# Socrates666/esp32-wake-word

Measured on AMD Instinct MI355X. Metric: audio windows/sec (1s@16kHz, 40-MFCC) through xiaoa CNN at 1/2/4/8 MI355X, higher is better.
Workload: dtype f32; 1 GPU; config2: fused MFCC(torchaudio+CMVN)+xiaoa CNN fp32, B clips per GPU; audio=fp32 samples, batch_per_gpu=65536, global_batch=65536, seq_len=16000, parallelism=dp1 (per-rank clip split, no collectives), process_group_world_size=1

## Files before the change

### esp32-wake-word_amd/csrc/wk_fused.hip

```cpp
#include "wk_fused_dev.h"

namespace {

#ifdef WK_DIAG
__device__ unsigned long long g_wk_stamps[16][16];
#endif

constexpr int kCnnCarve = kImgEnd - kGOff;
constexpr int kCnnLds = 2 * kCnnCarve;
static_assert(kCnnLds * 4 <= 163840, "standalone CNN LDS budget");
static_assert(kCnnCarve % 4 == 0 && kGOff % 4 == 0, "16-byte aligned carves");

template <int CM>
__global__ __launch_bounds__(kFusedBlock, 4) void wk_cnn_fused_kernel(const float* __restrict__ feats, int64_t batch,
                                                                     const float* __restrict__ wts,
                                                                     const uint16_t* __restrict__ wbf,
                                                                     float* __restrict__ logits, unsigned* err) {
  __shared__ __attribute__((aligned(16))) float smem[kCnnLds];
  const int tid = threadIdx.x, lane = tid & 63;
  const int wave = __builtin_amdgcn_readfirstlane(tid >> 6);
  for (int i = tid; i < kCnnLds; i += kFusedBlock) smem[i] = 0.0f;
  __syncthreads();
  const int role = wave >> 3;
  float* base = smem + role * kCnnCarve - kGOff;
  const int64_t cb = 2 * (int64_t)blockIdx.x + role, cs = 2 * (int64_t)gridDim.x;
  const int64_t n_mine = batch > cb ? (batch - 1 - cb) / cs + 1 : 0;
  FeatSrc<CM> src = {feats, base, cb, cs, 0};
  cnn_role<CM>(base, wts, wbf, n_mine, cb, cs, logits, wave & 7, lane, src);
  report_abort(reinterpret_cast<const unsigned*>(base + kCtrlOff), err, lane);
}

}

#ifdef WK_DIAG
extern "C" int wk_debug_stamps(unsigned long long* host_out, int reset) {
  if (hipMemcpyFromSymbol(host_out, HIP_SYMBOL(g_wk_stamps), sizeof(g_wk_stamps)) != hipSuccess) return 1;
  if (reset) {
    static unsigned long long zero[16][16];
    if (hipMemcpyToSymbol(HIP_SYMBOL(g_wk_stamps), zero, sizeof(zero)) != hipSuccess) return 1;
  }
  return 0;
}
#endif

namespace wk {

hipError_t launch_fused(bool i16, const void* audio, int64_t batch, int64_t clip_stride, const float* w,
                        const uint16_t* wbf, int conv_mode, float* logits, float* feats_or_null, int grid_cap,
                        hipStream_t stream, unsigned* err, int diag) {
  if (batch == 0) return hipSuccess;
  if (conv_mode != kConvF32 && !wbf) return hipErrorInvalidValue;
#ifdef WK_DIAG
  return launch_fused_modes<kConvBf16, kConvBf16x3, kConvF32>(i16, conv_mode, audio, batch, clip_stride, w, wbf, logits,
                                                              feats_or_null, grid_cap, stream, err, diag);
#else
  if (conv_mode != kConvF32)
    return launch_fused_xdl(i16, audio, batch, clip_stride, w, wbf, conv_mode, logits, feats_or_null, grid_cap, stream,
                            err, diag);
  return launch_fused_modes<kConvF32>(i16, conv_mode, audio, batch, clip_stride, w, wbf, logits, feats_or_null,
                                      grid_cap, stream, err, diag);
#endif
}

hipError_t launch_cnn_fused(const float* feats, int64_t batch, const float* w, const uint16_t* wbf, int conv_mode,
                            float* logits, int grid_cap, hipStream_t stream, unsigned* err) {
  if (batch == 0) return hipSuccess;
  if (conv_mode != kConvF32 && !wbf) return hipErrorInvalidValue;
  const int64_t roles = (batch + NBF - 1) / NBF;
  const int grid = (int)((roles + 1) / 2 < grid_cap ? (roles + 1) / 2 : grid_cap);
  if (conv_mode == kConvBf16)
    hipLaunchKernelGGL(wk_cnn_fused_kernel<kConvBf16>, dim3(grid), dim3(kFusedBlock), 0, stream, feats, batch, w, wbf,
                       logits, err);
  else if (conv_mode == kConvBf16x3)
    hipLaunchKernelGGL(wk_cnn_fused_kernel<kConvBf16x3>, dim3(grid), dim3(kFusedBlock), 0, stream, feats, batch, w,
                       wbf, logits, err);
  else
    hipLaunchKernelGGL(wk_cnn_fused_kernel<kConvF32>, dim3(grid), dim3(kFusedBlock), 0, stream, feats, batch, w, wbf,
                       logits, err);
  return hipGetLastError();
}

}
```

### esp32-wake-word_amd/csrc/wk_fused_cnn_role.h

```cpp
#pragma once
#include "wk_fused_lds.h"
#include "wk_cnn_dev.h"
#include "wk_kernels.h"

namespace {

__device__ __forceinline__ float row_sum16(float v) {
  v += dpp<0xB1>(v);
  v += dpp<0x4E>(v);
  v += dpp<0x141>(v);
  v += dpp<0x140>(v);
  return v;
}

template <int CM>
__device__ __forceinline__ void dct_cmvn_clip(const float* __restrict__ lbuf, int slot, float* __restrict__ F0,
                                              uint16_t* __restrict__ B0, uint16_t* __restrict__ X0,
                                              float* __restrict__ fo, int lane) {
  const int li = lane & 15, lk = lane >> 4;
  int aoff = 48 * lane;
  asm volatile("" : "+v"(aoff));
  const auto ra = make_rsrc(kDctB16, sizeof(kDctB16));
  float dA[12];
#pragma unroll
  for (int s = 0; s < 12; s += 4) {
    const f32x4 v = __builtin_bit_cast(f32x4, __builtin_amdgcn_raw_buffer_load_b128(ra, aoff, 4 * s, 0));
#pragma unroll
    for (int r = 0; r < 4; ++r) dA[s + r] = v[r];
  }
  f32x4 d[4] = {{0, 0, 0, 0}, {0, 0, 0, 0}, {0, 0, 0, 0}, {0, 0, 0, 0}};
#pragma unroll
  for (int s = 0; s < 10; ++s) {
    const f32x4 b = *reinterpret_cast<const f32x4*>(lbuf + (4 * s + lk) * WK_LSTRIDE + 4 * li);
#pragma unroll
    for (int nt = 0; nt < 4; ++nt) d[nt] = mfma4(dA[s], b[nt], d[nt]);
  }
  const bool v3 = li != 15;
  const int row0 = lane & 48;
#pragma unroll
  for (int r = 0; r < 4; ++r) {
    const float a = d[0][r];
    const float nx = __int_as_float(__builtin_amdgcn_update_dpp(__float_as_int(a), __float_as_int(a), 0x101, 0xF, 0xF, false));
    const bool ne = (a != d[1][r]) | (a != d[2][r]) | (v3 & (a != d[3][r])) | (a != nx);
    const bool flat = ((__builtin_amdgcn_ballot_w64(ne) >> row0) & 0xFFFFull) == 0;
#pragma unroll
    for (int nt = 0; nt < 4; ++nt) d[nt][r] = flat ? 0.0f : d[nt][r];
  }
  float mean[4], inv[4];
#pragma unroll
  for (int r = 0; r < 4; ++r) {
    const float x3 = v3 ? d[3][r] : 0.0f;
    mean[r] = row_sum16((d[0][r] + d[1][r]) + (d[2][r] + x3)) * (1.0f / kNFramesB);
    float dv[4];
#pragma unroll
    for (int nt = 0; nt < 4; ++nt) dv[nt] = d[nt][r] - mean[r];
    dv[3] = v3 ? dv[3] : 0.0f;
    const float q = row_sum16((dv[0] * dv[0] + dv[1] * dv[1]) + (dv[2] * dv[2] + dv[3] * dv[3]));
    float sd = __builtin_amdgcn_sqrtf(q * (1.0f / (kNFramesB - 1)));
    sd = sd == 0.0f ? 1.0f : sd;
    inv[r] = __builtin_amdgcn_rcpf(sd + 1e-8f);
  }
#pragma unroll
  for (int nt = 0; nt < 4; ++nt) {
    const int t = 4 * li + nt;
    if (nt == 3 && !v3) continue;
    const int row = slot * I0_TP + 1 + t;
    float y[4];
#pragma unroll
    for (int r = 0; r < 4; ++r) y[r] = (d[nt][r] - mean[r]) * inv[r];
    if constexpr (CM == kConvBf16) {
      uint2 pk;
      pk.x = bf16_bits(y[0]) | (bf16_bits(y[1]) << 16);
      pk.y = bf16_bits(y[2]) | (bf16_bits(y[3]) << 16);
      *reinterpret_cast<uint2*>(B0 + row * I0_CIP + 4 * lk) = pk;
    } else if constexpr (CM == kConvBf16x3) {
      uint32_t h[4], l[4];
#pragma unroll
      for (int r = 0; r < 4; ++r) {
        h[r] = bf16_bits(y[r]);
        l[r] = bf16_bits(y[r] - __uint_as_float(h[r] << 16));
      }
      *reinterpret_cast<uint2*>(X0 + row * X0_CIP + 4 * lk) = make_uint2(h[0] | (h[1] << 16), h[2] | (h[3] << 16));
      *reinterpret_cast<uint2*>(X0 + row * X0_CIP + 16 + 4 * lk) = make_uint2(l[0] | (l[1] << 16), l[2] | (l[3] << 16));
    } else {
      *reinterpret_cast<f32x4*>(F0 + row * F0_CIP + 4 * lk) = f32x4{y[0], y[1], y[2], y[3]};
    }
    if (fo) {
#pragma unroll
      for (int r = 0; r < 4; ++r)
        if (4 * lk + r < 13) fo[(4 * lk + r) * kNFramesB + t] = y[r];
    }
  }
}

template <int CM, class SRC>
__device__ __forceinline__ void cnn_role(float* base, const float* __restrict__ pk, const uint16_t* __restrict__ pkb,
                                         int64_t n_mine, int64_t clip_base, int64_t clip_step,
                                         float* __restrict__ logits, int cw, int lane, SRC& src) {
  float* F0 = base + kF0Off;
  float* F1 = base + kF1Off;
  float* F2 = base + kF2Off;
  uint16_t* B0 = reinterpret_cast<uint16_t*>(base + kB0Off);
  uint16_t* B1 = reinterpret_cast<uint16_t*>(base + kB1Off);
  uint16_t* B2 = reinterpret_cast<uint16_t*>(base + kB2Off);
  uint16_t* X0 = reinterpret_cast<uint16_t*>(base + kX0Off);
  uint16_t* X1 = reinterpret_cast<uint16_t*>(base + kX1Off);
  uint16_t* X2 = reinterpret_cast<uint16_t*>(base + kX2Off);
  constexpr bool BF = CM == kConvBf16, X3 = CM == kConvBf16x3;
  constexpr int kLoW = kNumPackedBf16;
  const auto rsb = make_rsrc(pkb, 2 * kNumPackedBf16 * (X3 ? 2 : 1));
  auto frag_bf = [&](int elem_off) -> s8 {
    return __builtin_bit_cast(s8, __builtin_amdgcn_raw_buffer_load_b128(rsb, 16 * lane, 2 * elem_off, 0));
  };
  float* Gp = base + kGOff;
  float* FCP = base + kFcpOff;
  unsigned* ctrl = reinterpret_cast<unsigned*>(base + kCtrlOff);
  const int li = lane & 15, lk = lane >> 4;
  unsigned gen = 0;
  const auto rs = make_rsrc(pk, 4 * kNumPacked);

  auto load_frags = [&](auto& w, int first) {
    constexpr int n = sizeof(w) / sizeof(float);
    static_assert(n % 4 == 0, "whole groups of four k-steps");
#pragma unroll
    for (int s = 0; s < n; s += 4) {
      const f32x4 v = __builtin_bit_cast(f32x4, __builtin_amdgcn_raw_buffer_load_b128(rs, 16 * lane, 4 * (first + s * 64), 0));
#pragma unroll
      for (int r = 0; r < 4; ++r) w[s + r] = v[r];
    }
  };
  float w3[48];
  s8 w3b[6];
  if constexpr (BF || X3) {
#pragma unroll
    for (int s = 0; s < 6; ++s) w3b[s] = frag_bf(kPbW3 + (cw * 6 + s) * kBfFrag);
  }
  if constexpr (CM == kConvF32) load_frags(w3, kPkW3 + cw * 48 * 64);
  const int64_t n_batches = (n_mine + NBF - 1) / NBF;
  src.init(cw, lane);
  bool eager_done = false;
  auto try_eager = [&](int64_t b) {
    if (cw >= NBF || eager_done) return;
    const int64_t i = (b + 1) * NBF + cw;
    if (i >= n_mine) return;
    if (src.ready(i)) {
      src.load(i, cw);
      eager_done = true;
    }
  };
  auto fc2 = [&](int64_t bb) {
    if (cw != 0) return;
    int ln = lane;
    asm volatile("" : "+v"(ln));
    const int cl = ln & (NBF - 1), q = ln >> 2;
    float h[4];
    if constexpr (CM == kConvF32) {
      f32x4 v = *reinterpret_cast<const f32x4*>(FCP + cl * 64 + 4 * q);
#pragma unroll
      for (int w = 1; w < 8; ++w) v += *reinterpret_cast<const f32x4*>(FCP + (w * NBF + cl) * 64 + 4 * q);
#pragma unroll
      for (int r = 0; r < 4; ++r) h[r] = v[r];
    } else {
      const f32x4 v = *reinterpret_cast<const f32x4*>(FCP + cl * 64 + 4 * q);
#pragma unroll
      for (int r = 0; r < 4; ++r) h[r] = v[r];
#pragma unroll
      for (int w = 1; w < 8; ++w) {
        const f32x4 u = *reinterpret_cast<const f32x4*>(FCP + (w * NBF + cl) * 64 + 4 * q);
#pragma unroll
        for (int r = 0; r < 4; ++r) h[r] += u[r];
      }
    }
    float acc = 0.0f;
#pragma unroll
    for (int i2 = 0; i2 < 4; ++i2) acc = __builtin_fmaf(buf_load(rs, 16 * q, 4 * (kPkF2 + i2)), fmaxf(h[i2], 0.0f), acc);
    acc += __shfl_xor(acc, 4, 64);
    acc += __shfl_xor(acc, 8, 64);
    acc += __shfl_xor(acc, 16, 64);
    acc += __shfl_xor(acc, 32, 64);
    const int64_t i = bb * NBF + cl;
    if (q == 0 && i < n_mine) logits[clip_base + clip_step * i] = acc;
  };
  WK_STAMP_INIT
  for (int64_t b = 0; b < n_batches; ++b) {
    if (cw < NBF && !eager_done) {
      const int64_t i = b * NBF + cw;
      if (i < n_mine) {
        src.wait(i);
        src.load(i, cw);
      }
    }
    eager_done = false;
    float w1[12];
    s8 w1b[2], w1l[2];
    if constexpr (BF || X3) {
#pragma unroll
      for (int s = 0; s < 2; ++s) w1b[s] = frag_bf(kPbW1 + ((cw & 1) * 2 + s) * kBfFrag);
    }
    if constexpr (X3) {
#pragma unroll
      for (int s = 0; s < 2; ++s) w1l[s] = frag_bf(kLoW + kPbW1 + ((cw & 1) * 2 + s) * kBfFrag);
    }
    if constexpr (CM == kConvF32) load_frags(w1, kPkW1 + (cw & 1) * 12 * 64);
    WK_STAMP(0);
    role_sync<0>(ctrl, kCtrlCnnBar, gen, lane);
    if (b > 0) fc2(b - 1);

    const int nv = n_mine - b * NBF < NBF ? (int)(n_mine - b * NBF) : NBF;

    if ((cw >> 1) < nv) {
      const int co0 = 16 * (cw & 1), cl = cw >> 1;
      const int bo = (cl * I0_TP + li) * I0_CIP;
#pragma unroll 1
      for (int p = 0; p < 2; ++p) {
        const int ta = 32 * p, tb = ta + 16;
        f32x4 acc_a = {0, 0, 0, 0}, acc_b = {0, 0, 0, 0};
        if constexpr (BF) {
          conv_pair_bf<2, 16, I0_CIP>(B0, w1b, bo + ta * I0_CIP, bo + tb * I0_CIP, lk, acc_a, acc_b);
          epi_pool_bf<I1_CIP, I1_TP, 31>(acc_a, B1, co0, cl, ta, lane);
          epi_pool_bf<I1_CIP, I1_TP, 31>(acc_b, B1, co0, cl, tb, lane);
        } else if constexpr (X3) {
          const int bx = (cl * I0_TP + li) * X0_CIP;
          conv_pair_bf3<2, 16, X0_CIP>(X0, w1b, w1l, bx + ta * X0_CIP, bx + tb * X0_CIP, lk, acc_a, acc_b);
          epi_pool_bf3<X1_CIP, I1_TP, 31, 32>(acc_a, X1, co0, cl, ta, lane);
          epi_pool_bf3<X1_CIP, I1_TP, 31, 32>(acc_b, X1, co0, cl, tb, lane);
        } else {
          f32x4 m[4] = {{0, 0, 0, 0}, {0, 0, 0, 0}, {0, 0, 0, 0}, {0, 0, 0, 0}};
          conv_wino_v<1, F0_CIP>(F0, w1, (cl * I0_TP + 2 * (16 * p + li)) * F0_CIP + 4 * lk, m);
          epi_wino_pool<F1_CIP, I1_TP, 31>(m, F1, co0, cl, 16 * p, lane);
        }
      }
    }
    WK_STAMP(1);
    role_sync<0>(ctrl, kCtrlCnnBar, gen, lane);
    try_eager(b);
    WK_STAMP(2);

    if constexpr (BF) {
      s8 w2b[3];
#pragma unroll
      for (int s = 0; s < 3; ++s) w2b[s] = frag_bf(kPbW2 + ((cw & 3) * 3 + s) * kBfFrag);
      const int co0 = 16 * (cw & 3);
#pragma unroll 1
      for (int p = 0; p < 2; ++p) {
        const int cl = 2 * (cw >> 2) + p;
        if (cl >= nv) break;
        const int bb = (cl * I1_TP + li) * I1_CIP;
        f32x4 acc_a = {0, 0, 0, 0}, acc_b = {0, 0, 0, 0};
        conv_pair_bf<3, 32, I1_CIP>(B1, w2b, bb, bb + 16 * I1_CIP, lk, acc_a, acc_b);
        epi_pool_bf<I2_CIP, I2_TP, 15>(acc_a, B2, co0, cl, 0, lane);
        epi_pool_bf<I2_CIP, I2_TP, 15>(acc_b, B2, co0, cl, 16, lane);
      }
    } else if constexpr (X3) {
      s8 w2b[3], w2l[3];
#pragma unroll
      for (int s = 0; s < 3; ++s) w2b[s] = frag_bf(kPbW2 + ((cw & 3) * 3 + s) * kBfFrag);
#pragma unroll
      for (int s = 0; s < 3; ++s) w2l[s] = frag_bf(kLoW + kPbW2 + ((cw & 3) * 3 + s) * kBfFrag);
      const int co0 = 16 * (cw & 3);
#pragma unroll 1
      for (int p = 0; p < 2; ++p) {
        const int cl = 2 * (cw >> 2) + p;
        if (cl >= nv) break;
        const int bb = (cl * I1_TP + li) * X1_CIP;
        f32x4 acc_a = {0, 0, 0, 0}, acc_b = {0, 0, 0, 0};
        conv_pair_bf3<3, 32, X1_CIP>(X1, w2b, w2l, bb, bb + 16 * X1_CIP, lk, acc_a, acc_b);
        epi_pool_bf3<X2_CIP, I2_TP, 15, 64>(acc_a, X2, co0, cl, 0, lane);
        epi_pool_bf3<X2_CIP, I2_TP, 15, 64>(acc_b, X2, co0, cl, 16, lane);
      }
    } else {
      float w2[24];
      load_frags(w2, kPkW2 + (cw & 3) * 24 * 64);
      const int co0 = 16 * (cw & 3);
#pragma unroll 1
      for (int p = 0; p < 2; ++p) {
        const int cl = 2 * (cw >> 2) + p;
        if (cl >= nv) break;
        f32x4 m[4] = {{0, 0, 0, 0}, {0, 0, 0, 0}, {0, 0, 0, 0}, {0, 0, 0, 0}};
        conv_wino_v<2, F1_CIP, 1>(F1, w2, (cl * I1_TP + 2 * li) * F1_CIP + 4 * lk, m);
        epi_wino_pool<F2_CIP, I2_TP, 15>(m, F2, co0, cl, 0, lane);
      }
    }
    WK_STAMP(3);
    role_sync<0>(ctrl, kCtrlCnnBar, gen, lane);
    try_eager(b);
    WK_STAMP(4);

    {
      const int co0 = 16 * cw;
      const int bo = li * I2_CIP;
#pragma unroll 1
      for (int p = 0; p < 2; ++p) {
        if (p > 0) try_eager(b);
        const int ca = 2 * p, cb = 2 * p + 1;
        if (ca >= nv) break;
        f32x4 acc_a = {0, 0, 0, 0}, acc_b = {0, 0, 0, 0};
        if constexpr (BF) {
          conv_pair_bf<6, 64, I2_CIP, 3>(B2, w3b, bo + ca * I2_TP * I2_CIP, bo + cb * I2_TP * I2_CIP, lk, acc_a,
                                         acc_b);
        } else if constexpr (X3) {
          s8 w3l[6];
#pragma unroll
          for (int s = 0; s < 6; ++s) w3l[s] = frag_bf(kLoW + kPbW3 + (cw * 6 + s) * kBfFrag);
          const int bx = li * X2_CIP;
          conv_pair_bf3<6, 64, X2_CIP, 2>(X2, w3b, w3l, bx + ca * I2_TP * X2_CIP, bx + cb * I2_TP * X2_CIP, lk,
                                          acc_a, acc_b);
        } else {
          f32x4 m[4] = {{0, 0, 0, 0}, {0, 0, 0, 0}, {0, 0, 0, 0}, {0, 0, 0, 0}};
          conv_wino_v<4, F2_CIP, 1>(F2, w3, ((ca + (li >> 3)) * I2_TP + 2 * (li & 7)) * F2_CIP + 4 * lk, m);
          epi_wino_gap<NBF>(m, Gp, co0, ca, lane);
          continue;
        }
        epi_gap<NBF>(acc_a, Gp, co0, ca, lane);
        epi_gap<NBF>(acc_b, Gp, co0, cb, lane);
      }
    }
    float wf1[16];
    load_frags(wf1, kPkF1 + cw * 16 * 64);
    WK_STAMP(5);
    role_sync<0>(ctrl, kCtrlCnnBar, gen, lane);
    try_eager(b);
    WK_STAMP(6);

    {
      int ln = lane;
      asm volatile("" : "+v"(ln));
      f32x4 acc = {0, 0, 0, 0};
      const float* g = Gp + 16 * cw * NBF + (ln & (NBF - 1));
#pragma unroll
      for (int s = 0; s < 16; ++s) acc = mfma4x4(wf1[s], g[s * NBF], acc);
      *reinterpret_cast<f32x4*>(FCP + (cw * NBF + (ln & (NBF - 1))) * 64 + 4 * (ln >> 2)) = acc;
    }
    try_eager(b);
    WK_STAMP(8);
  }
  if (n_batches > 0) {
    role_sync<0>(ctrl, kCtrlCnnBar, gen, lane);
    fc2(n_batches - 1);
  }
  WK_STAMP_FLUSH(8 + cw);
}

template <int CM, bool FEATS>
struct LogmelSrc {
  float* smem;
  unsigned* ctrl;
  float* feats_out;
  int64_t clip_base, clip_step;
  int cw, lane, diag;
  __device__ __forceinline__ void init(int cw_, int lane_) {
    cw = cw_;
    lane = lane_;
    signal_set(ctrl, kCtrlLFree + cw, cw < NBF ? (unsigned)cw : 0xFFFFFFFFu, lane);
  }
  __device__ __forceinline__ bool ready(int64_t i) const {
    __atomic_signal_fence(__ATOMIC_SEQ_CST);
    const bool r = (diag & 2) ||
                   __builtin_amdgcn_readfirstlane(lds_load(ctrl + kCtrlLReady)) >= 8u * (unsigned)(i + 1);
    asm volatile("" ::: "memory");
    __atomic_signal_fence(__ATOMIC_SEQ_CST);
    return r;
  }
  __device__ __forceinline__ void wait(int64_t i) const {
    if (!(diag & 2)) spin_until<0>(ctrl, kCtrlLReady, 8u * (unsigned)(i + 1));
  }
  __device__ __forceinline__ void load(int64_t i, int slot) const {
    float* fo = FEATS ? feats_out + (clip_base + clip_step * i) * (13 * kNFramesB) : nullptr;
    dct_cmvn_clip<CM>(smem + (i & 1 ? kL1Off : kLOff), slot, smem + kF0Off,
                      reinterpret_cast<uint16_t*>(smem + kB0Off), reinterpret_cast<uint16_t*>(smem + kX0Off), fo,
                      lane);
    signal_set(ctrl, kCtrlLFree + cw, (unsigned)(i + NBF), lane);
  }
};

template <int CM>
struct FeatSrc {
  const float* feats;
  float* base;
  int64_t clip_base, clip_step;
  int lane;
  __device__ __forceinline__ void init(int, int lane_) { lane = lane_; }
  __device__ __forceinline__ bool ready(int64_t) const { return true; }
  __device__ __forceinline__ void wait(int64_t) const {}
  __device__ __forceinline__ void load(int64_t i, int slot) const {
    const float* f = feats + (clip_base + clip_step * i) * (13 * kNFramesB);
    if (lane >= kNFramesB) return;
    float y[13];
#pragma unroll
    for (int c = 0; c < 13; ++c) y[c] = __builtin_nontemporal_load(f + c * kNFramesB + lane);
    const int row = slot * I0_TP + 1 + lane;
    if constexpr (CM == kConvBf16) {
      uint16_t* B0 = reinterpret_cast<uint16_t*>(base + kB0Off) + row * I0_CIP;
#pragma unroll
      for (int c = 0; c < 12; c += 4)
        *reinterpret_cast<uint2*>(B0 + c) = make_uint2(bf16_bits(y[c]) | (bf16_bits(y[c + 1]) << 16),
                                                       bf16_bits(y[c + 2]) | (bf16_bits(y[c + 3]) << 16));
      B0[12] = (uint16_t)bf16_bits(y[12]);
    } else if constexpr (CM == kConvBf16x3) {
      uint16_t* X0 = reinterpret_cast<uint16_t*>(base + kX0Off) + row * X0_CIP;
#pragma unroll
      for (int c = 0; c < 13; ++c) {
        const uint32_t h = bf16_bits(y[c]);
        X0[c] = (uint16_t)h;
        X0[16 + c] = (uint16_t)bf16_bits(y[c] - __uint_as_float(h << 16));
      }
    } else {
      float* F0 = base + kF0Off + row * F0_CIP;
#pragma unroll
      for (int c = 0; c < 12; c += 4) *reinterpret_cast<f32x4*>(F0 + c) = f32x4{y[c], y[c + 1], y[c + 2], y[c + 3]};
      F0[12] = y[12];
    }
  }
};

}
```

### esp32-wake-word_amd/csrc/wk_fused_dev.h

```cpp
#pragma once
#include "wk_fused_lds.h"
#include "wk_fused_fe_role.h"
#include "wk_fused_cnn_role.h"
#include "wk_kernels.h"
#include <type_traits>

namespace {

template <typename T, int CM, bool FEATS>
__global__ __launch_bounds__(kFusedBlock, 4) void wk_fused_kernel(const T* __restrict__ audio, int64_t batch,
                                                                 int64_t clip_stride, const float* __restrict__ wts,
                                                                 const uint16_t* __restrict__ wbf,
                                                                 float* __restrict__ logits,
                                                                 float* __restrict__ feats_out, unsigned* err,
                                                                 int diag) {
  __shared__ __attribute__((aligned(16))) float smem[kFusedLds];
#ifndef WK_DIAG
  diag = 0;
#endif
  const int tid = threadIdx.x;
  const int lane = tid & 63;
  const int wave = __builtin_amdgcn_readfirstlane(tid >> 6);
  typedef std::conditional_t<CM == kConvF32, FePacked, FeScalar> FE;
  fe_init_tables<true, true, FE>(smem, tid, kFusedBlock);
  for (int i = tid; i < kFusedLds - kGOff; i += kFusedBlock) smem[kGOff + i] = 0.0f;
  __syncthreads();
  const int64_t n_mine = batch > (int64_t)blockIdx.x ? (batch - 1 - blockIdx.x) / gridDim.x + 1 : 0;
  if (wave < kFeWaves) __builtin_amdgcn_s_setprio(kPrioFe);
  if (wave < kFeWaves) {
    if (!(diag & 2)) fe_role<T, FE>(smem, audio, n_mine, clip_stride, wave, lane, diag);
  } else {
    if (!(diag & 1)) {
      LogmelSrc<CM, FEATS> src = {smem, reinterpret_cast<unsigned*>(smem + kCtrlOff), feats_out, (int64_t)blockIdx.x,
                                  (int64_t)gridDim.x, 0, 0, diag};
      cnn_role<CM>(smem, wts, wbf, n_mine, (int64_t)blockIdx.x, (int64_t)gridDim.x, logits, wave - kFeWaves, lane,
                   src);
    }
  }
  report_abort(reinterpret_cast<unsigned*>(smem + kCtrlOff), err, lane);
}

template <typename T, int CM>
hipError_t launch_fused_as(const void* audio, int64_t batch, int64_t clip_stride, const float* w, const uint16_t* wbf,
                           float* logits, float* feats_or_null, int grid_cap, hipStream_t stream, unsigned* err,
                           int diag) {
  const dim3 g((int)(batch < grid_cap ? batch : grid_cap)), blk(kFusedBlock);
  if (feats_or_null)
    hipLaunchKernelGGL((wk_fused_kernel<T, CM, true>), g, blk, 0, stream, (const T*)audio, batch, clip_stride, w, wbf,
                       logits, feats_or_null, err, diag);
  else
    hipLaunchKernelGGL((wk_fused_kernel<T, CM, false>), g, blk, 0, stream, (const T*)audio, batch, clip_stride, w, wbf,
                       logits, nullptr, err, diag);
  return hipGetLastError();
}

template <typename T, int CM, int... REST, typename... A>
hipError_t launch_fused_mode(int conv_mode, A... a) {
  if constexpr (sizeof...(REST) > 0)
    return conv_mode == CM ? launch_fused_as<T, CM>(a...) : launch_fused_mode<T, REST...>(conv_mode, a...);
  else
    return launch_fused_as<T, CM>(a...);
}
template <int... CMS, typename... A>
hipError_t launch_fused_modes(bool i16, int conv_mode, A... a) {
  return i16 ? launch_fused_mode<int16_t, CMS...>(conv_mode, a...) : launch_fused_mode<float, CMS...>(conv_mode, a...);
}

}
```

### esp32-wake-word_amd/csrc/wk_fused_fe_role.h

```cpp
#pragma once
#include "wk_fused_lds.h"

namespace {

template <typename T, typename FE>
__device__ __forceinline__ void fe_role(float* smem, const T* __restrict__ audio, int64_t n_mine,
                                        int64_t clip_stride, int wave, int lane, int diag) {
  float* P = smem + kPOff;
  float* L = smem + kLOff;
  float* L1 = smem + kL1Off;
  unsigned* ctrl = reinterpret_cast<unsigned*>(smem + kCtrlOff);
  const int g = lane >> 4, j = lane & 15;
  const FeTables tb = fe_tables(smem, j, nullptr);
  const int slot_base = fe_lds::slot_base(g);
  const int64_t G = gridDim.x;
  unsigned gen = 0, p_wait = 0;

  const int64_t step = G * clip_stride;
  const T* cptr = audio + (int64_t)blockIdx.x * clip_stride;
  constexpr uint32_t kClipBytes = kWinSamples * sizeof(T);
  struct PfCtx {
    __amdgpu_buffer_rsrc_t rs;
    int base;
    int xb;
  };
  auto fwr = [&](int r) { return FE::round1_swap && r == 1 ? wave ^ 4 : wave; };
  auto pf_ctx = [&](const T* p, bool ok, int r) -> PfCtx {
    const int fl = fwr(r) + fe_lds::kRoundSlots * r + slot_base;
    return {make_rsrc(p, ok ? kClipBytes : 0u), 256 * fl - 160, fl == 0 ? 160 : 256 * fl - 161};
  };

  Raw<T> pf;
  {
    const PfCtx c0 = pf_ctx(cptr, n_mine > 0, 0);
#pragma unroll
    for (int k = 0; k < 4; ++k) load_raw_part<FE>(c0.rs, c0.base, c0.xb, j, pf, k);
  }
  WK_STAMP_INIT
  for (int64_t i = 0; i < n_mine; ++i) {
#pragma unroll 1
    for (int r = 0; r <= 1; ++r) {
      const int fl = fwr(r) + fe_lds::kRoundSlots * r + slot_base;
      const int edge = r == 0 && fwr(r) == 0 ? 1 : r == 1 && fwr(r) == 6 ? 2 : 0;
      typename FE::c2 a[16];
#ifdef WK_DIAG
      asm volatile("s_waitcnt vmcnt(0)" ::: "memory");
      WK_STAMP(11);
#endif
      fe_stage0_fused(pf, lane, edge, tb, a);
      WK_STAMP(0);
      const PfCtx nx = r < 1 ? pf_ctx(cptr, true, r + 1) : pf_ctx(cptr + step, i + 1 < n_mine, 0);
      auto pf_part = [&](int k) {
        if (k >= 0) {
          load_raw_part<FE>(nx.rs, nx.base, nx.xb, j, pf, k);
        } else if (r == 0) {
          spin_until<kPrioFe>(ctrl, kCtrlFeBar, p_wait);
          WK_STAMP(9);
        }
      };
      WK_STAMP(1);
      float* row = fl < kNFramesB ? P + fl * kPRow : smem + kDummyRowOff;
      fe_rest<true, FE>(a, j, row, tb, 0, pf_part WK_SP_ARG);
    }
    role_sync<kPrioFe>(ctrl, kCtrlFeBar, gen, lane);
    WK_STAMP(7);
    if (i >= 2 && !(diag & 1)) spin_until_all8<kPrioFe>(ctrl, kCtrlLFree, (unsigned)(i - 1));
    WK_STAMP(10);
    {
      int prow = kPOff + min(lane, kNFramesB - 1) * kPRow;
      asm volatile("" : "+v"(prow));
      mel_dispatch<true>(wave, smem + prow, (i & 1 ? L1 : L) + lane);
      WK_STAMP(8);
      signal_add(ctrl, kCtrlLReady, lane);
    }
    gen += 8;
    signal_add(ctrl, kCtrlFeBar, lane);
    p_wait = gen;
    cptr += step;
  }
  WK_STAMP_FLUSH(wave);
}

}
```

### esp32-wake-word_amd/csrc/wk_fused_lds.h

```cpp
#pragma once
#include "wk_fe_dev.h"

using namespace wk;

namespace {

#ifdef WK_DIAG
extern __device__ unsigned long long g_wk_stamps[16][16];
#define WK_STAMP_INIT WkStamps _stamps; _stamps.init();
#define WK_STAMP(k) _stamps.hit(k)
#define WK_STAMP_FLUSH(w) do { if (lane == 0) for (int _k = 0; _k < 16; ++_k) atomicAdd(&g_wk_stamps[w][_k], _stamps.st[_k]); } while (0)
#define WK_SP_ARG , &_stamps
#else
#define WK_STAMP_INIT
#define WK_STAMP(k) do {} while (0)
#define WK_STAMP_FLUSH(w) do {} while (0)
#define WK_SP_ARG
#endif

constexpr int NBF = 4;
constexpr int kFeWaves = 8;
constexpr int kFusedBlock = 1024;
constexpr int kGOff = (kFeLds + 3) & ~3;
constexpr int kFcpOff = kGOff + 128 * NBF;
constexpr int kFcpSize = 8 * NBF * 64;
constexpr int kL1Off = kFcpOff + kFcpSize;
static_assert(kLOff % 4 == 0 && kL1Off % 4 == 0, "log-mel buffers are read with ds_read_b128");
constexpr int kCtrlOff = kL1Off + kLSize;
constexpr int kImgOff = (kCtrlOff + 16 + 3) & ~3;
constexpr int I0_CIP = 24, I1_CIP = 40, I2_CIP = 72;
constexpr int I0_TP = 64, I1_TP = 32, I2_TP = 18;
constexpr int F0_CIP = 20, F1_CIP = 36, F2_CIP = 68;
constexpr int kF0Off = kImgOff;
constexpr int kF1Off = kF0Off + NBF * I0_TP * F0_CIP;
constexpr int kF2Off = kF1Off + NBF * I1_TP * F1_CIP;
constexpr int kF2End = kF2Off + NBF * I2_TP * F2_CIP;
constexpr int kImgEnd = kImgOff + NBF * (I0_TP * 40 + I1_TP * 72 + I2_TP * 136) / 2 > kF2End
                            ? kImgOff + NBF * (I0_TP * 40 + I1_TP * 72 + I2_TP * 136) / 2
                            : kF2End;
constexpr int kB0Off = kImgOff;
constexpr int kB1Off = kB0Off + NBF * I0_TP * I0_CIP / 2;
constexpr int kB2Off = kB1Off + NBF * I1_TP * I1_CIP / 2;
constexpr int X0_CIP = 40, X1_CIP = 72, X2_CIP = 136;
constexpr int kX0Off = kImgOff;
constexpr int kX1Off = kX0Off + NBF * I0_TP * X0_CIP / 2;
constexpr int kX2Off = kX1Off + NBF * I1_TP * X1_CIP / 2;
static_assert(kX2Off + NBF * I2_TP * X2_CIP / 2 <= kImgEnd, "split images fit the fp32 carve");
static_assert(kF1Off % 4 == 0 && kF2Off % 4 == 0 && kB1Off % 2 == 0 && kB2Off % 2 == 0 && kX1Off % 2 == 0 &&
                  kX2Off % 2 == 0, "vector-aligned images");
enum { kConvF32 = 0, kConvBf16 = 1, kConvBf16x3 = 2 };
constexpr int kDummyRowOff = (kImgEnd + 1) & ~1;
constexpr int kFusedLds = kDummyRowOff + kPRow;
static_assert(kFusedLds * 4 <= 163840, "fused LDS budget");
static_assert(kPOff + kPSize <= kGOff && kLOff + kLSize <= kPOff && kImgEnd <= kDummyRowOff,
              "CNN carve disjoint from the front-end's power rows, log-mel buffer and dummy row");
static_assert(kGOff + 128 * NBF <= kFcpOff && kFcpOff + kFcpSize <= kL1Off && kL1Off + kLSize <= kCtrlOff &&
                  kCtrlOff + 16 <= kImgOff,
              "pooled features | partials | log-mel buffer 1 | control words, in that order, disjoint");
static_assert(kF2End <= kImgEnd && kB2Off + NBF * I2_TP * I2_CIP / 2 <= kImgEnd &&
                  kX2Off + NBF * I2_TP * X2_CIP / 2 <= kImgEnd,
              "every precision's conv images end inside [kImgOff, kImgEnd)");

enum { kCtrlFeBar = 0, kCtrlCnnBar = 1, kCtrlLReady = 2, kCtrlLFree = 4, kCtrlAbort = 15 };
static_assert(kCtrlOff % 4 == 0 && kCtrlLFree % 4 == 0, "spin_until_all8 reads the eight LFree words as two uint4");
constexpr unsigned kSpinLimit = 1u << 22;

__device__ __forceinline__ unsigned lds_load(const unsigned* p) {
  return __hip_atomic_load(p, __ATOMIC_RELAXED, __HIP_MEMORY_SCOPE_WORKGROUP);
}
__device__ __forceinline__ unsigned lds_load_u(const unsigned* p) {
  return __builtin_amdgcn_readfirstlane(lds_load(p));
}

constexpr int kPrioFe = 3;
constexpr int kSpinSleep = 2;

template <int PRIO, typename F>
__device__ __forceinline__ void spin_on(unsigned* ctrl, const F& ready) {
  __atomic_signal_fence(__ATOMIC_SEQ_CST);
  if (!ready()) {
    if (PRIO > 0) __builtin_amdgcn_s_setprio(0);
    for (unsigned n = 4;; n += 4) {
      __builtin_amdgcn_s_sleep(kSpinSleep);
      if (ready()) break;
      __builtin_amdgcn_s_sleep(kSpinSleep);
      if (ready()) break;
      __builtin_amdgcn_s_sleep(kSpinSleep);
      if (ready()) break;
      __builtin_amdgcn_s_sleep(kSpinSleep);
      if (ready()) break;
      if ((n & 31) == 0 && (n >= kSpinLimit || lds_load_u(ctrl + kCtrlAbort))) {
        __hip_atomic_store(ctrl + kCtrlAbort, 1u, __ATOMIC_RELAXED, __HIP_MEMORY_SCOPE_WORKGROUP);
        break;
      }
    }
    if (PRIO > 0) __builtin_amdgcn_s_setprio(PRIO);
  }
  asm volatile("" ::: "memory");
  __atomic_signal_fence(__ATOMIC_SEQ_CST);
}

template <int PRIO>
__device__ __forceinline__ void spin_until(unsigned* ctrl, int idx, unsigned v) {
  spin_on<PRIO>(ctrl, [=] { return lds_load_u(ctrl + idx) >= v; });
}

template <int PRIO>
__device__ __forceinline__ void role_sync(unsigned* ctrl, int idx, unsigned& gen, int lane) {
  gen += 8;
  __atomic_signal_fence(__ATOMIC_SEQ_CST);
  asm volatile("s_waitcnt lgkmcnt(0)" ::: "memory");
  if (lane == 0) __hip_atomic_fetch_add(ctrl + idx, 1u, __ATOMIC_RELAXED, __HIP_MEMORY_SCOPE_WORKGROUP);
  spin_until<PRIO>(ctrl, idx, gen);
}

__device__ __forceinline__ unsigned min8(const unsigned* ctrl, int idx) {
  asm volatile("" ::: "memory");
  const uint4* q = reinterpret_cast<const uint4*>(ctrl + idx);
  const uint4 a = q[0], b = q[1];
  return min(min(min(a.x, a.y), min(a.z, a.w)), min(min(b.x, b.y), min(b.z, b.w)));
}
template <int PRIO>
__device__ __forceinline__ void spin_until_all8(unsigned* ctrl, int idx, unsigned v) {
  spin_on<PRIO>(ctrl, [=] { return __builtin_amdgcn_readfirstlane(min8(ctrl, idx)) >= v; });
}

__device__ __forceinline__ void signal_set(unsigned* ctrl, int idx, unsigned v, int lane) {
  __atomic_signal_fence(__ATOMIC_SEQ_CST);
  asm volatile("s_waitcnt lgkmcnt(0)" ::: "memory");
  if (lane == 0) __hip_atomic_store(ctrl + idx, v, __ATOMIC_RELAXED, __HIP_MEMORY_SCOPE_WORKGROUP);
  __atomic_signal_fence(__ATOMIC_SEQ_CST);
}

__device__ __forceinline__ void signal_add(unsigned* ctrl, int idx, int lane) {
  __atomic_signal_fence(__ATOMIC_SEQ_CST);
  asm volatile("s_waitcnt lgkmcnt(0)" ::: "memory");
  if (lane == 0) __hip_atomic_fetch_add(ctrl + idx, 1u, __ATOMIC_RELAXED, __HIP_MEMORY_SCOPE_WORKGROUP);
  __atomic_signal_fence(__ATOMIC_SEQ_CST);
}

__device__ __forceinline__ void report_abort(const unsigned* ctrl, unsigned* err, int lane) {
  if (lane == 0 && err) {
    const unsigned ab = lds_load(ctrl + kCtrlAbort);
    if (ab) __hip_atomic_store(err, ab == 1u ? 1u : 3u, __ATOMIC_RELAXED, __HIP_MEMORY_SCOPE_SYSTEM);
  }
}

}
```

Baseline: 36.64 million windows/s.

## Triple-buffer log-mel ring by moving pooled features and partials into conv images

Adds a third log-mel buffer so the front-end waves can run one more clip ahead of the CNN waves before waiting on LFree. The LDS space for it comes from relocating the pooled features (G) and classifier partials (FCP) into otherwise-dead rows of the conv2/conv3 images, keeping the total LDS carve size unchanged. It also disables the mid-conv3 eager load for the bf16 mode. The aliasing adds risk of data races if those image rows are read while G/FCP are live, and the static asserts are what guard that.

```diff
diff --git a/esp32-wake-word_amd/csrc/wk_fused.hip b/esp32-wake-word_amd/csrc/wk_fused.hip
--- a/esp32-wake-word_amd/csrc/wk_fused.hip
+++ b/esp32-wake-word_amd/csrc/wk_fused.hip
@@ -6,10 +6,10 @@
 __device__ unsigned long long g_wk_stamps[16][16];
 #endif
 
-constexpr int kCnnCarve = kImgEnd - kGOff;
+constexpr int kCnnCarve = kImgEnd - kCnnWinOff;
 constexpr int kCnnLds = 2 * kCnnCarve;
 static_assert(kCnnLds * 4 <= 163840, "standalone CNN LDS budget");
-static_assert(kCnnCarve % 4 == 0 && kGOff % 4 == 0, "16-byte aligned carves");
+static_assert(kCnnCarve % 4 == 0 && kCnnWinOff % 4 == 0, "16-byte aligned carves");
 
 template <int CM>
 __global__ __launch_bounds__(kFusedBlock, 4) void wk_cnn_fused_kernel(const float* __restrict__ feats, int64_t batch,
@@ -22,7 +22,7 @@
   for (int i = tid; i < kCnnLds; i += kFusedBlock) smem[i] = 0.0f;
   __syncthreads();
   const int role = wave >> 3;
-  float* base = smem + role * kCnnCarve - kGOff;
+  float* base = smem + role * kCnnCarve - kCnnWinOff;
   const int64_t cb = 2 * (int64_t)blockIdx.x + role, cs = 2 * (int64_t)gridDim.x;
   const int64_t n_mine = batch > cb ? (batch - 1 - cb) / cs + 1 : 0;
   FeatSrc<CM> src = {feats, base, cb, cs, 0};
diff --git a/esp32-wake-word_amd/csrc/wk_fused_cnn_role.h b/esp32-wake-word_amd/csrc/wk_fused_cnn_role.h
--- a/esp32-wake-word_amd/csrc/wk_fused_cnn_role.h
+++ b/esp32-wake-word_amd/csrc/wk_fused_cnn_role.h
@@ -93,6 +93,7 @@
   }
 }
 
+constexpr bool kEagerMidConv3[3] = {true, false, true};
 template <int CM, class SRC>
 __device__ __forceinline__ void cnn_role(float* base, const float* __restrict__ pk, const uint16_t* __restrict__ pkb,
                                          int64_t n_mine, int64_t clip_base, int64_t clip_step,
@@ -112,8 +113,8 @@
   auto frag_bf = [&](int elem_off) -> s8 {
     return __builtin_bit_cast(s8, __builtin_amdgcn_raw_buffer_load_b128(rsb, 16 * lane, 2 * elem_off, 0));
   };
-  float* Gp = base + kGOff;
-  float* FCP = base + kFcpOff;
+  float* Gp = base + g_off(CM);
+  float* FCP = base + fcp_off(CM);
   unsigned* ctrl = reinterpret_cast<unsigned*>(base + kCtrlOff);
   const int li = lane & 15, lk = lane >> 4;
   unsigned gen = 0;
@@ -157,7 +158,7 @@
     if constexpr (CM == kConvF32) {
       f32x4 v = *reinterpret_cast<const f32x4*>(FCP + cl * 64 + 4 * q);
 #pragma unroll
-      for (int w = 1; w < 8; ++w) v += *reinterpret_cast<const f32x4*>(FCP + (w * NBF + cl) * 64 + 4 * q);
+      for (int w = 1; w < 8; ++w) v += *reinterpret_cast<const f32x4*>(FCP + fcp_at(CM, w, 0) + cl * 64 + 4 * q);
 #pragma unroll
       for (int r = 0; r < 4; ++r) h[r] = v[r];
     } else {
@@ -166,7 +167,7 @@
       for (int r = 0; r < 4; ++r) h[r] = v[r];
 #pragma unroll
       for (int w = 1; w < 8; ++w) {
-        const f32x4 u = *reinterpret_cast<const f32x4*>(FCP + (w * NBF + cl) * 64 + 4 * q);
+        const f32x4 u = *reinterpret_cast<const f32x4*>(FCP + fcp_at(CM, w, 0) + cl * 64 + 4 * q);
 #pragma unroll
         for (int r = 0; r < 4; ++r) h[r] += u[r];
       }
@@ -291,7 +292,7 @@
       const int bo = li * I2_CIP;
 #pragma unroll 1
       for (int p = 0; p < 2; ++p) {
-        if (p > 0) try_eager(b);
+        if (p > 0 && kEagerMidConv3[CM]) try_eager(b);
         const int ca = 2 * p, cb = 2 * p + 1;
         if (ca >= nv) break;
         f32x4 acc_a = {0, 0, 0, 0}, acc_b = {0, 0, 0, 0};
@@ -329,7 +330,7 @@
       const float* g = Gp + 16 * cw * NBF + (ln & (NBF - 1));
 #pragma unroll
       for (int s = 0; s < 16; ++s) acc = mfma4x4(wf1[s], g[s * NBF], acc);
-      *reinterpret_cast<f32x4*>(FCP + (cw * NBF + (ln & (NBF - 1))) * 64 + 4 * (ln >> 2)) = acc;
+      *reinterpret_cast<f32x4*>(FCP + fcp_at(CM, cw, 0) + (ln & (NBF - 1)) * 64 + 4 * (ln >> 2)) = acc;
     }
     try_eager(b);
     WK_STAMP(8);
@@ -348,9 +349,11 @@
   float* feats_out;
   int64_t clip_base, clip_step;
   int cw, lane, diag;
+  int lk3;
   __device__ __forceinline__ void init(int cw_, int lane_) {
     cw = cw_;
     lane = lane_;
+    lk3 = cw_ == 3 ? 0 : cw_;
     signal_set(ctrl, kCtrlLFree + cw, cw < NBF ? (unsigned)cw : 0xFFFFFFFFu, lane);
   }
   __device__ __forceinline__ bool ready(int64_t i) const {
@@ -364,9 +367,11 @@
   __device__ __forceinline__ void wait(int64_t i) const {
     if (!(diag & 2)) spin_until<0>(ctrl, kCtrlLReady, 8u * (unsigned)(i + 1));
   }
-  __device__ __forceinline__ void load(int64_t i, int slot) const {
+  __device__ __forceinline__ void load(int64_t i, int slot) {
     float* fo = FEATS ? feats_out + (clip_base + clip_step * i) * (13 * kNFramesB) : nullptr;
-    dct_cmvn_clip<CM>(smem + (i & 1 ? kL1Off : kLOff), slot, smem + kF0Off,
+    const int lo = lring_off(lk3);
+    lk3 = lring_next(lk3);
+    dct_cmvn_clip<CM>(smem + lo, slot, smem + kF0Off,
                       reinterpret_cast<uint16_t*>(smem + kB0Off), reinterpret_cast<uint16_t*>(smem + kX0Off), fo,
                       lane);
     signal_set(ctrl, kCtrlLFree + cw, (unsigned)(i + NBF), lane);
diff --git a/esp32-wake-word_amd/csrc/wk_fused_dev.h b/esp32-wake-word_amd/csrc/wk_fused_dev.h
--- a/esp32-wake-word_amd/csrc/wk_fused_dev.h
+++ b/esp32-wake-word_amd/csrc/wk_fused_dev.h
@@ -23,7 +23,7 @@
   const int wave = __builtin_amdgcn_readfirstlane(tid >> 6);
   typedef std::conditional_t<CM == kConvF32, FePacked, FeScalar> FE;
   fe_init_tables<true, true, FE>(smem, tid, kFusedBlock);
-  for (int i = tid; i < kFusedLds - kGOff; i += kFusedBlock) smem[kGOff + i] = 0.0f;
+  for (int i = tid; i < kFusedLds - kCnnWinOff; i += kFusedBlock) smem[kCnnWinOff + i] = 0.0f;
   __syncthreads();
   const int64_t n_mine = batch > (int64_t)blockIdx.x ? (batch - 1 - blockIdx.x) / gridDim.x + 1 : 0;
   if (wave < kFeWaves) __builtin_amdgcn_s_setprio(kPrioFe);
diff --git a/esp32-wake-word_amd/csrc/wk_fused_fe_role.h b/esp32-wake-word_amd/csrc/wk_fused_fe_role.h
--- a/esp32-wake-word_amd/csrc/wk_fused_fe_role.h
+++ b/esp32-wake-word_amd/csrc/wk_fused_fe_role.h
@@ -7,14 +7,13 @@
 __device__ __forceinline__ void fe_role(float* smem, const T* __restrict__ audio, int64_t n_mine,
                                         int64_t clip_stride, int wave, int lane, int diag) {
   float* P = smem + kPOff;
-  float* L = smem + kLOff;
-  float* L1 = smem + kL1Off;
   unsigned* ctrl = reinterpret_cast<unsigned*>(smem + kCtrlOff);
   const int g = lane >> 4, j = lane & 15;
   const FeTables tb = fe_tables(smem, j, nullptr);
   const int slot_base = fe_lds::slot_base(g);
   const int64_t G = gridDim.x;
   unsigned gen = 0, p_wait = 0;
+  int lk3 = 0;
 
   const int64_t step = G * clip_stride;
   const T* cptr = audio + (int64_t)blockIdx.x * clip_stride;
@@ -64,12 +63,13 @@
     }
     role_sync<kPrioFe>(ctrl, kCtrlFeBar, gen, lane);
     WK_STAMP(7);
-    if (i >= 2 && !(diag & 1)) spin_until_all8<kPrioFe>(ctrl, kCtrlLFree, (unsigned)(i - 1));
+    if (i >= 3 && !(diag & 5)) spin_until_all8<kPrioFe>(ctrl, kCtrlLFree, (unsigned)(i - 2));
     WK_STAMP(10);
     {
       int prow = kPOff + min(lane, kNFramesB - 1) * kPRow;
       asm volatile("" : "+v"(prow));
-      mel_dispatch<true>(wave, smem + prow, (i & 1 ? L1 : L) + lane);
+      mel_dispatch<true>(wave, smem + prow, smem + lring_off(lk3) + lane);
+      lk3 = lring_next(lk3);
       WK_STAMP(8);
       signal_add(ctrl, kCtrlLReady, lane);
     }
diff --git a/esp32-wake-word_amd/csrc/wk_fused_lds.h b/esp32-wake-word_amd/csrc/wk_fused_lds.h
--- a/esp32-wake-word_amd/csrc/wk_fused_lds.h
+++ b/esp32-wake-word_amd/csrc/wk_fused_lds.h
@@ -1,5 +1,6 @@
 #pragma once
 #include "wk_fe_dev.h"
+#include "wk_fused_lds_layout.h"
 
 using namespace wk;
 
@@ -18,45 +19,19 @@
 #define WK_SP_ARG
 #endif
 
-constexpr int NBF = 4;
+using namespace wk::fused_lds;
+static_assert(kLStride == WK_LSTRIDE && kFrames == kNFramesB && kPowerRow == kPRow && kFeEnd == kFeLds &&
+                  kFeL0Off == kLOff && kLFloats == kLSize,
+              "wk_fused_lds_layout.h restates the front-end's constants");
 constexpr int kFeWaves = 8;
 constexpr int kFusedBlock = 1024;
-constexpr int kGOff = (kFeLds + 3) & ~3;
-constexpr int kFcpOff = kGOff + 128 * NBF;
-constexpr int kFcpSize = 8 * NBF * 64;
-constexpr int kL1Off = kFcpOff + kFcpSize;
-static_assert(kLOff % 4 == 0 && kL1Off % 4 == 0, "log-mel buffers are read with ds_read_b128");
-constexpr int kCtrlOff = kL1Off + kLSize;
-constexpr int kImgOff = (kCtrlOff + 16 + 3) & ~3;
-constexpr int I0_CIP = 24, I1_CIP = 40, I2_CIP = 72;
-constexpr int I0_TP = 64, I1_TP = 32, I2_TP = 18;
-constexpr int F0_CIP = 20, F1_CIP = 36, F2_CIP = 68;
-constexpr int kF0Off = kImgOff;
-constexpr int kF1Off = kF0Off + NBF * I0_TP * F0_CIP;
-constexpr int kF2Off = kF1Off + NBF * I1_TP * F1_CIP;
-constexpr int kF2End = kF2Off + NBF * I2_TP * F2_CIP;
-constexpr int kImgEnd = kImgOff + NBF * (I0_TP * 40 + I1_TP * 72 + I2_TP * 136) / 2 > kF2End
-                            ? kImgOff + NBF * (I0_TP * 40 + I1_TP * 72 + I2_TP * 136) / 2
-                            : kF2End;
-constexpr int kB0Off = kImgOff;
-constexpr int kB1Off = kB0Off + NBF * I0_TP * I0_CIP / 2;
-constexpr int kB2Off = kB1Off + NBF * I1_TP * I1_CIP / 2;
-constexpr int X0_CIP = 40, X1_CIP = 72, X2_CIP = 136;
-constexpr int kX0Off = kImgOff;
-constexpr int kX1Off = kX0Off + NBF * I0_TP * X0_CIP / 2;
-constexpr int kX2Off = kX1Off + NBF * I1_TP * X1_CIP / 2;
-static_assert(kX2Off + NBF * I2_TP * X2_CIP / 2 <= kImgEnd, "split images fit the fp32 carve");
-static_assert(kF1Off % 4 == 0 && kF2Off % 4 == 0 && kB1Off % 2 == 0 && kB2Off % 2 == 0 && kX1Off % 2 == 0 &&
-                  kX2Off % 2 == 0, "vector-aligned images");
-enum { kConvF32 = 0, kConvBf16 = 1, kConvBf16x3 = 2 };
-constexpr int kDummyRowOff = (kImgEnd + 1) & ~1;
-constexpr int kFusedLds = kDummyRowOff + kPRow;
 static_assert(kFusedLds * 4 <= 163840, "fused LDS budget");
-static_assert(kPOff + kPSize <= kGOff && kLOff + kLSize <= kPOff && kImgEnd <= kDummyRowOff,
-              "CNN carve disjoint from the front-end's power rows, log-mel buffer and dummy row");
-static_assert(kGOff + 128 * NBF <= kFcpOff && kFcpOff + kFcpSize <= kL1Off && kL1Off + kLSize <= kCtrlOff &&
-                  kCtrlOff + 16 <= kImgOff,
-              "pooled features | partials | log-mel buffer 1 | control words, in that order, disjoint");
+__device__ __forceinline__ constexpr int lring_off(int k) { return k == 0 ? kLOff : k == 1 ? kL1Off : kL2Off; }
+__device__ __forceinline__ constexpr int lring_next(int k) { return k == 2 ? 0 : k + 1; }
+static_assert(kPOff + kPSize <= kCnnWinOff && kLOff + kLSize <= kPOff && kImgEnd <= kDummyRowOff,
+              "CNN carve disjoint from the front-end's power rows, log-mel buffer 0 and dummy row");
+static_assert(kL2Off + kLSize <= kL1Off && kL1Off + kLSize <= kCtrlOff && kCtrlOff + 16 <= kImgOff,
+              "log-mel buffer 2 | log-mel buffer 1 | control words | images, in that order, disjoint");
 static_assert(kF2End <= kImgEnd && kB2Off + NBF * I2_TP * I2_CIP / 2 <= kImgEnd &&
                   kX2Off + NBF * I2_TP * X2_CIP / 2 <= kImgEnd,
               "every precision's conv images end inside [kImgOff, kImgEnd)");
diff --git a/esp32-wake-word_amd/csrc/wk_fused_lds_layout.h b/esp32-wake-word_amd/csrc/wk_fused_lds_layout.h
--- /dev/null
+++ b/esp32-wake-word_amd/csrc/wk_fused_lds_layout.h
@@ -0,0 +1,100 @@
+#pragma once
+#include "wk_fe_lds_layout.h"
+
+namespace wk {
+namespace fused_lds {
+
+constexpr int kLStride = 64, kFrames = 63, kPowerRow = 270;
+constexpr int kFeEnd = fe_lds::carve(kLStride, kFrames, kPowerRow).end;
+constexpr int kFeL0Off = fe_lds::carve(kLStride, kFrames, kPowerRow).logmel;
+constexpr int kLFloats = 40 * kLStride;
+constexpr int kLimitBytes = fe_lds::kFusedLimitBytes;
+
+constexpr int NBF = 4;
+constexpr int kGFloats = 128 * NBF;
+constexpr int kFcpGroup = 2 * NBF * 64;
+constexpr int kFcpFloats = 4 * kFcpGroup;
+
+constexpr int kCnnWinOff = (kFeEnd + 3) & ~3;
+constexpr int kL2Off = kCnnWinOff;
+constexpr int kL1Off = kL2Off + kLFloats;
+constexpr int kCtrlOff = kL1Off + kLFloats;
+constexpr int kImgOff = (kCtrlOff + 16 + 3) & ~3;
+
+constexpr int I0_TP = 64, I1_TP = 32, I2_TP = 18;
+constexpr int I0_L = 63, I1_L = 31, I2_L = 15;
+constexpr int I0_CIP = 24, I1_CIP = 40, I2_CIP = 72;
+constexpr int X0_CIP = 40, X1_CIP = 72, X2_CIP = 136;
+constexpr int F0_CIP = 20, F1_CIP = 36, F2_CIP = 68;
+
+enum { kConvF32 = 0, kConvBf16 = 1, kConvBf16x3 = 2 };
+
+struct Images {
+  int off[3], pitch[3], end;
+};
+constexpr Images images(int p0, int p1, int p2) {
+  Images m = {};
+  m.pitch[0] = p0, m.pitch[1] = p1, m.pitch[2] = p2;
+  m.off[0] = kImgOff;
+  m.off[1] = m.off[0] + NBF * I0_TP * p0;
+  m.off[2] = m.off[1] + NBF * I1_TP * p1;
+  m.end = m.off[2] + NBF * I2_TP * p2;
+  return m;
+}
+constexpr Images images(int cm) {
+  return cm == kConvF32    ? images(F0_CIP, F1_CIP, F2_CIP)
+         : cm == kConvBf16 ? images(I0_CIP / 2, I1_CIP / 2, I2_CIP / 2)
+                           : images(X0_CIP / 2, X1_CIP / 2, X2_CIP / 2);
+}
+static_assert(I0_CIP % 2 == 0 && I1_CIP % 2 == 0 && I2_CIP % 2 == 0 && X0_CIP % 2 == 0 && X1_CIP % 2 == 0 &&
+                  X2_CIP % 2 == 0, "bf16 rows are whole floats");
+
+constexpr int kF0Off = images(kConvF32).off[0], kF1Off = images(kConvF32).off[1], kF2Off = images(kConvF32).off[2];
+constexpr int kB0Off = images(kConvBf16).off[0], kB1Off = images(kConvBf16).off[1], kB2Off = images(kConvBf16).off[2];
+constexpr int kX0Off = images(kConvBf16x3).off[0], kX1Off = images(kConvBf16x3).off[1],
+              kX2Off = images(kConvBf16x3).off[2];
+constexpr int kF2End = images(kConvF32).end;
+constexpr int max3(int a, int b, int c) { return a > b ? (a > c ? a : c) : (b > c ? b : c); }
+constexpr int kImgEnd = max3(images(kConvF32).end, images(kConvBf16).end, images(kConvBf16x3).end);
+
+constexpr int g_off(int cm) { return images(cm).off[1] + images(cm).pitch[1]; }
+constexpr int fcp_off(int cm) { return images(cm).off[2] + images(cm).pitch[2]; }
+constexpr int fcp_stride(int cm) { return I2_TP * images(cm).pitch[2]; }
+constexpr int fcp_at(int cm, int w, int cl) { return (w >> 1) * fcp_stride(cm) + ((w & 1) * NBF + cl) * 64; }
+
+constexpr int rows_begin(int cm, int l, int c) {
+  return images(cm).off[l] + (c * (l == 0 ? I0_TP : l == 1 ? I1_TP : I2_TP) + 1) * images(cm).pitch[l];
+}
+constexpr int rows_end(int cm, int l, int c) {
+  return rows_begin(cm, l, c) + (l == 0 ? I0_L : l == 1 ? I1_L : I2_L) * images(cm).pitch[l];
+}
+constexpr bool g_ok(int cm) {
+  return g_off(cm) % 4 == 0 && g_off(cm) >= rows_begin(cm, 1, 0) && g_off(cm) + kGFloats <= rows_end(cm, 1, 0);
+}
+constexpr bool fcp_ok(int cm) {
+  for (int c = 0; c < NBF; ++c) {
+    const int a = fcp_off(cm) + fcp_at(cm, 2 * c, 0);
+    if (a % 4 || a < rows_begin(cm, 2, c) || a + kFcpGroup > rows_end(cm, 2, c)) return false;
+    if (fcp_at(cm, 2 * c + 1, NBF - 1) + 64 != fcp_at(cm, 2 * c, 0) + kFcpGroup) return false;
+  }
+  return true;
+}
+static_assert(g_ok(kConvF32) && g_ok(kConvBf16) && g_ok(kConvBf16x3),
+              "pooled features: inside the data rows of conv2-image clip 0, 16-byte aligned");
+static_assert(fcp_ok(kConvF32) && fcp_ok(kConvBf16) && fcp_ok(kConvBf16x3),
+              "classifier.0 partials: 512 floats inside the data rows of each conv3-image clip, 16-byte aligned");
+static_assert(rows_end(kConvBf16, 2, 0) - rows_begin(kConvBf16, 2, 0) == 540 && kFcpGroup == 512,
+              "plain bf16: the partials of two k-slices fit one conv3 clip with 28 floats to spare");
+static_assert(kGFloats + kFcpFloats == kLFloats && kL2Off + kGFloats + kFcpFloats == kL1Off,
+              "the third log-mel buffer is exactly the former pooled-features | partials range");
+static_assert(kFeL0Off % 4 == 0 && kL1Off % 4 == 0 && kL2Off % 4 == 0, "log-mel buffers are read with ds_read_b128");
+static_assert(kF1Off % 4 == 0 && kF2Off % 4 == 0 && kB1Off % 2 == 0 && kB2Off % 2 == 0 && kX1Off % 2 == 0 &&
+                  kX2Off % 2 == 0, "vector-aligned images");
+
+constexpr int kDummyRowOff = (kImgEnd + 1) & ~1;
+constexpr int kFusedLds = kDummyRowOff + kPowerRow;
+static_assert(kFusedLds * 4 <= kLimitBytes, "fused LDS budget");
+static_assert(kFusedLds * 4 == 163016, "the carve's total is what it was with two log-mel buffers");
+
+}
+}
```

Result: no change. 36.81 million windows/s, median of 6 (+0.4%).
